# xp3i4/linear

Measured on AMD Instinct MI355X. Metric: reads/sec (whole node) + HBM GB/s on seed lookup, 10 kb reads vs GRCh38, higher is better.
Workload: dtype u64

## Files before the change

### linear_amd/csrc/lnr_api.hip

```cpp
#include <cstring>
#include <rocprim/device/device_radix_sort.hpp>
#include "lnr_kernels.hip"
#include "lnr_gap_args.h"
#include "../../include/linear_amd.h"

#include <algorithm>
#include <dlfcn.h>
#include <chrono>
#include <cstdio>
#include <cstdlib>
#include <atomic>
#include <condition_variable>
#include <deque>
#include <memory>
#include <mutex>
#include <string>
#include <thread>
#include <vector>

using namespace lnr;

#include "lnr_host_util.h"
#include "lnr_ctx.h"
#include "lnr_index.h"
// ... 176 lines not shown
        case LNR_ERR_NO_DEVICE: return "no usable HIP device (this library has no CPU path)";
        case LNR_ERR_HIP: return "HIP runtime error";
        case LNR_ERR_NOMEM: return "out of memory";
        case LNR_ERR_NO_INDEX: return "index not built";
        case LNR_ERR_LIMIT: return "input exceeds a format limit";
        case LNR_ERR_UNSUPPORTED: return "option not supported by this build";
        case LNR_ERR_INTERNAL: return "internal capacity overflow";
    }
    return "unknown status";
}
const char *lnr_last_error(const lnr_ctx *ctx) { return ctx ? const_cast<lnr_ctx *>(ctx)->err.show() : "null context"; }

lnr_status lnr_create(const lnr_opts *opts, lnr_ctx **out) {
    if (!out) return LNR_ERR_ARG;
    *out = nullptr;
    lnr_opts o;
    if (opts) o = *opts; else lnr_opts_default(&o);
    if ((o.index_type != 1 && o.index_type != 2) || o.feature_type != 2 || (o.preset != 1 && o.preset != 2) || o.dup > 1) return LNR_ERR_UNSUPPORTED;
    int ndev = 0;
    if (hipGetDeviceCount(&ndev) != hipSuccess || ndev <= 0) { (void)hipGetLastError(); return LNR_ERR_NO_DEVICE; }
    int dev = o.device;
    if (dev < 0) { if (hipGetDevice(&dev) != hipSuccess) return LNR_ERR_NO_DEVICE; }
    if (dev >= ndev) return LNR_ERR_ARG;
    int prev_dev = -1;
    (void)hipGetDevice(&prev_dev);
    if (hipSetDevice(dev) != hipSuccess) return LNR_ERR_NO_DEVICE;
    struct Restore { int d; ~Restore() { if (d >= 0) (void)hipSetDevice(d); } } restore_{prev_dev == dev ? -1 : prev_dev};
    lnr_ctx *ctx = new (std::nothrow) lnr_ctx();
    if (!ctx) return LNR_ERR_NOMEM;
    ctx->opts = o;
    ctx->device = dev;
    ctx->tun = tuning_from_env(dev);
    ctx->lane1_nomem_test = ctx->tun.lane1_nomem;
    ctx->lane[0] = lane_create(ctx, 0);
    bool ok = ctx->lane[0] && ctx->s_copy.create() && ctx->s_down.create() && ctx->ev_down.create() == hipSuccess && ctx->ev_done.create() == hipSuccess;
    if (!ok) { (void)hipGetLastError(); lnr_destroy(ctx); return LNR_ERR_HIP; }
    *out = ctx;
    return LNR_OK;
}

void lnr_destroy(lnr_ctx *ctx) {
    if (!ctx) return;
    (void)hipSetDevice(ctx->device);
    { std::lock_guard<std::mutex> g(ctx->mu); ctx->quit = true; }
    ctx->cv.notify_all();
    for (auto &L : ctx->lane) if (L && L->th.joinable()) L->th.join();
    ctx->s_copy.sync(); ctx->s_down.sync();
    delete ctx;
}

lnr_status lnr_filter_batch_dev(lnr_ctx *ctx, const uint8_t *d_reads, const uint64_t *d_off, uint32_t n, lnr_cords_dev *out) {
    if (!ctx || !d_off || (n && !d_reads)) return LNR_ERR_ARG;
    DevGuard dg_(ctx->device);
    if (in_flight(ctx)) { ctx->err = "batches submitted with lnr_filter_submit are still in flight"; return LNR_ERR_ARG; }
    return lane0_result(ctx, filter_dev(ctx->lane[0].get(), d_reads, d_off, n, out));
}
lnr_status lnr_last_gaps(lnr_ctx *ctx, lnr_gaps *out) {
    if (!ctx || !out) return LNR_ERR_ARG;
    DevGuard dg_(ctx->device);
    if (!ctx->tickets.empty()) { ctx->err = "lnr_last_gaps: batches are in flight (a worker is writing the per-read arrays)"; return LNR_ERR_ARG; }
    Lane *L = ctx->lane[0].get();
    u32 n = L->last_n;
    out->n_reads = n; out->n_gaps = 0; out->gap_off = nullptr; out->gaps = nullptr;
    ctx->h_gap_off.assign((size_t)n + 1, 0);
    ctx->h_gap_pairs.clear();
    if (n && L->last_gaps_off.size() == n) {
// ... 193 lines not shown
```

### linear_amd/csrc/lnr_ctx.h

```cpp
#pragma once
#include "lnr_handover.h"

struct lnr_ctx;

namespace {

struct Index {
    bool has_index = false;
    lnr_index_info info{};
    std::vector<u64> seq_len, seq_off, f2_off;
    u32 nbins = 0;
    DevBuf g, dir, hs, f2, d_seq_off, d_f2_off, d_seq_len;
    DevBuf bm, bl, ov;
    DevBuf hx_nkeys, hx_nvals; u32 hx_nnodes = 0; u64 hx_empty_dir = 0;
};

struct Tuning {
    size_t job_lds_bytes = 6 * 1024;
    u32 heavy_lds_kb = 48;
    u32 mid_cap = 6144, mid_lds_kb = 24;
    u32 heavy_cap = 0xffffffffu;
    u32 heavy_cap_r1 = 7000, mid_cap_r1 = 3000;
    u32 stop_after = 0;
    u32 mid_waves = 0;
    bool mid_cap_env = false;
    int seed_bm = -1;
    u32 prep_threads = 256;
    u32 prep_grid = 4096;
    u32 bulk_delay_ticks = 10000;
    u32 cap_shrink = 1;
    u32 seed_lds_pad = 0;
    u32 gap_arena2_mb = 64;
    u32 gap_teams = 96, ncu = 0;
    u32 gap_heavy_w = 60000;
    u64 gap_work_cap = 3000000;
    u32 nlanes = 2;
    int lane1_prio = 1;
    bool lane1_nomem = false;
    bool handover_gate = true;
    u64 gaps_spec = 0;
};

Tuning tuning_from_env(int device) {
    Tuning t;
    if (const char *e = getenv("LNR_LANES")) { long v = atol(e); if (v == 1 || v == 2) t.nlanes = (u32)v; }
    if (const char *e = getenv("LNR_LANE1_NOMEM")) t.lane1_nomem = atoi(e) != 0;
    if (const char *e = getenv("LNR_HANDOVER_GATE")) t.handover_gate = atoi(e) != 0;
    if (const char *e = getenv("LNR_GAPS_SPEC")) { long long v = atoll(e); if (v >= 1) t.gaps_spec = (u64)v; }
    if (const char *e = getenv("LNR_LANE1_PRIO")) { long v = atol(e); if (v >= -1 && v <= 1) t.lane1_prio = (int)v; }
    if (const char *e = getenv("LNR_CAP_SHRINK")) { long v = atol(e); if (v >= 1 && v <= 4096) t.cap_shrink = (u32)v; }
    if (const char *e = getenv("LNR_GAP_TEAMS")) { long v = atol(e); if (v >= 1 && v <= 4096) t.gap_teams = (u32)v; }
// ... 125 lines not shown
```

### linear_amd/csrc/lnr_hd.h

```cpp
#pragma once
#include <stdint.h>
#include <limits.h>
#include "ref_sort.h"

namespace lnr {

typedef uint64_t u64;
typedef int64_t i64;
typedef uint32_t u32;
typedef int32_t i32;
typedef uint16_t u16;
typedef uint8_t u8;

struct UP { u64 first, second; };

#if defined(__HIP_DEVICE_COMPILE__)
#define LNR_GLOBAL __attribute__((address_space(1)))
#define LNR_LDS __attribute__((address_space(3)))
#else
#define LNR_GLOBAL
#define LNR_LDS
#endif
template <class T> LNR_HD inline LNR_GLOBAL T *as_global(T *p) { return (LNR_GLOBAL T *)p; }
template <class T> LNR_HD inline LNR_LDS T *as_lds(T *p) { return (LNR_LDS T *)p; }

static const u64 ANCHOR_ZERO = 1ULL << 20;
static const u64 F_END = 1ULL << 60, F_STRAND = 1ULL << 61, F_RECD = 1ULL << 62, F_MAIN = 1ULL << 63;
static const u64 VALUE_MASK_DSTR = ((1ULL << 60) - 1) | F_STRAND;
static const u64 MAX_CORD_ID = (1ULL << 10) - 1, MAX_CORD_X = (1ULL << 30) - 1;

LNR_HD inline u64 cord_x(u64 v) { return (v >> 20) & ((1ULL << 30) - 1); }
LNR_HD inline u64 cord_y(u64 v) { return v & 0xfffffULL; }
LNR_HD inline u64 cord_strand(u64 v) { return (v >> 61) & 1ULL; }
LNR_HD inline u64 cord_id(u64 v) { return (v >> 50) & 1023ULL; }
LNR_HD inline u64 cord_x40(u64 v) { return (v >> 20) & 0xffffffffffULL; }
LNR_HD inline u64 mk_cord(u64 idx, u64 y, u64 s) { return (idx << 20) + y + (s << 61); }
// ... 13 lines not shown
}
LNR_HD inline UP forward_y(UP se, u64 L) {
    UP r;
    if (cord_strand(se.first)) { r.first = L - cord_y(se.second) - 1; r.second = L - cord_y(se.first) - 1; }
    else { r.first = cord_y(se.first); r.second = cord_y(se.second); }
    return r;
}

LNR_HD inline bool lnr_is_leader() {
#if defined(__HIP_DEVICE_COMPILE__)
    return (threadIdx.x & 63) == 0;
#else
    return true;
#endif
}
LNR_HD inline void lnr_wave_sync() {
#if defined(__HIP_DEVICE_COMPILE__)
    __builtin_amdgcn_fence(__ATOMIC_RELEASE, "workgroup");
    __builtin_amdgcn_wave_barrier();
    __builtin_amdgcn_fence(__ATOMIC_ACQUIRE, "workgroup");
#endif
}
LNR_HD inline u32 lnr_uni32(u32 v) {
#if defined(__HIP_DEVICE_COMPILE__)
    return (u32)__builtin_amdgcn_readfirstlane((int)v);
#else
    return v;
#endif
}
LNR_HD inline u64 lnr_uni64(u64 v) { return ((u64)lnr_uni32((u32)(v >> 32)) << 32) | (u64)lnr_uni32((u32)v); }
template <class T, class P = T *>
struct Vec {
    P p; u32 n, cap; int *ovf;
    LNR_HD void init(P p_, u32 cap_, int *ovf_) { p = p_; n = 0; cap = cap_; ovf = ovf_; }
    LNR_HD void push(const T &v) { if (n < cap) p[n++] = v; else *ovf = 1; }
    LNR_HD void push_u(const T &v) {
        if (n < cap) { if (lnr_is_leader()) p[n] = v; n++; }
        else if (lnr_is_leader()) *ovf = 1;
    }
    LNR_HD T &operator[](u32 i) { return p[i]; }
    LNR_HD T &back() { return p[n - 1]; }
};
struct Arena {
    char *base; u64 off, cap; int ovf; Arena *next;
    LNR_HD void init(void *b, u64 c) { base = (char *)b; off = 0; cap = c; ovf = 0; next = nullptr; }
    template <class T> LNR_HD T *get(u64 n) {
        u64 bytes = (n * sizeof(T) + 15) & ~15ULL;
        Arena *a = this;
        while (a->off + bytes > a->cap) {
            if (!a->next) { a->ovf = 1; ovf = 1; return (T *)base; }
            a = a->next;
        }
        T *r = (T *)(a->base + a->off);
        a->off += bytes;
        return r;
    }
};
struct Arena1 {
    char *base; u64 off, cap; int ovf;
    LNR_HD void init(void *b, u64 c) { base = (char *)b; off = 0; cap = c; ovf = 0; }
    template <class T> LNR_HD T *get(u64 n) {
        u64 bytes = (n * sizeof(T) + 15) & ~15ULL;
        if (off + bytes > cap) { ovf = 1; return (T *)base; }
        T *r = (T *)(base + off);
        off += bytes;
        return r;
    }
};
LNR_HD inline u64 job_scratch_bytes(u64 cap) { return (cap + 2) * 160 + 1024; }
LNR_HD inline u64 tail_scratch_bytes(u64 cap) { return cap * 240 + 8192; }

LNR_HD inline int lnr_popc64(u64 v) {
#if defined(__HIP_DEVICE_COMPILE__)
    return __popcll(v);
#else
    return __builtin_popcountll(v);
#endif
}
struct PackedSeq {
    const u64 *pk; const u32 *nm; u64 L;
    LNR_HD u8 operator[](u64 i) const {
        u64 j = i < L ? i : L;
        u32 n = nm[j >> 5]; u64 w = pk[j >> 5];
        u32 v = (u32)(w >> (2 * (j & 31))) & 3;
        return (u8)(((n >> (j & 31)) & 1) ? 4 : v);
    }
    LNR_HD int sum20(u64 p) const {
        u64 w = p >> 5; u32 sh = (u32)(p & 31);
// ... 873 lines not shown
#else
template <class FV, class CV>
LNR_HD inline bool extend_window(FV f1, FV f2, CV &cords, u64 &tail, u64 cordy_str, u64 cordy_end) {
    u32 p_str = cords.n - 1;
    u64 nc;
    while ((nc = previous_window(f1, f2, tail)) && cord_y(nc) >= cordy_str) {
        if (cords.n >= cords.cap) { *cords.ovf = 1; return false; }
        cords.push(nc); tail = nc;
    }
    u32 p_end = cords.n;
    if (p_end - p_str > 1) {
        for (u32 k = p_str; k < (p_str + p_end) / 2; k++) rs_swap(cords[k], cords[cords.n - k + p_str - 1]);
        tail = cords[cords.n - 1];
    }
    while ((nc = next_window(f1, f2, tail)) && cord_y(nc) + 96 < cordy_end) {
        if (cords.n >= cords.cap) { *cords.ovf = 1; return false; }
        cords.push(nc); tail = nc;
    }
    return true;
}
#endif
template <class FP, class OP> struct GenomeFeatT { FP base; OP off; u32 nseq; };
typedef GenomeFeatT<const F96 *, const u64 *> GenomeFeat;
typedef GenomeFeatT<LNR_GLOBAL const F96 *, LNR_GLOBAL const u64 *> GGenomeFeat;
template <class FP, class OP>
LNR_HD inline FeatViewT<FP> f2_view(GenomeFeatT<FP, OP> g, u64 id) {
    FeatViewT<FP> v;
    if (id >= g.nseq) { v.p = g.base; v.n = 0; return v; }
    v.p = g.base + g.off[id]; v.n = (u32)(g.off[id + 1] - g.off[id]);
    return v;
}
template <class FV, class GF>
LNR_HD inline void filter_hits_flags(const u64 *hits, u32 nhits, const FV f1[2], GF g, i32 *keep, u32 first, u32 step) {
    for (u32 it = 1 + first; it < nhits; it += step) {
        u32 dist = wdist_checked(f1[cord_strand(hits[it])], f2_view(g, cord_id(hits[it])), cord_y(hits[it]) >> 4, cord_x(hits[it]) >> 4);
        keep[it] = dist < 50 ? 1 : 0;
    }
}
LNR_HD inline u32 filter_hits_apply(u64 *hits, u32 nhits, const i32 *keep) {
    u32 mv = 0;
    for (u32 it = 1; it < nhits; it++) {
        if (keep[it]) hits[it - mv] = hits[it];
        else mv++;
        if (is_end(hits[it])) hits[it - mv] |= F_END;
    }
    return nhits - mv;
}
template <class FV, class GF, class CV>
LNR_HD inline void path_dst_2(const u64 *hits, u32 nhits, const FV f1_[2], GF g, CV &cords_, u64 read_str, u64 read_end, u64 L) {
    i64 hitBegin = 1, hitEnd = (i64)nhits;
    if (hitBegin >= hitEnd - 1) return;
    CV cords = cords_;
    struct NBack { CV &dst; CV &src; LNR_HD ~NBack() { dst.n = src.n; } } nback_{cords_, cords};
    FV f1[2] = {f1_[0], f1_[1]};
    cords.p = (decltype(cords.p))lnr_uni64((u64)cords.p); cords.n = lnr_uni32(cords.n); cords.cap = lnr_uni32(cords.cap); cords.ovf = (int *)lnr_uni64((u64)cords.ovf);
    for (int k = 0; k < 2; k++) { f1[k].p = (decltype(f1[k].p))lnr_uni64((u64)f1[k].p); f1[k].n = lnr_uni32(f1[k].n); }
    g.base = (decltype(g.base))lnr_uni64((u64)g.base); g.off = (decltype(g.off))lnr_uni64((u64)g.off); g.nseq = lnr_uni32(g.nseq);
    read_str = lnr_uni64(read_str); read_end = lnr_uni64(read_end); L = lnr_uni64(L);
    hitEnd = (i64)lnr_uni32(nhits);
    u64 tail;
    if (cords.n == 0) { cords.push_u(F_END); tail = F_END; }
    else tail = lnr_uni64(cords.p[cords.n - 1]);
    u64 ready_str, ready_end, cordy_str = 0, cordy_end = 0;
    bool f_sp_l, f_sp_r = false, f_block_end = false, f_append;
    i64 itt_next = hitBegin + 1, itt_first = hitBegin;
#if defined(LNR_PROF) && defined(__HIP_DEVICE_COMPILE__)
    unsigned long long pdc_[12] = {0, 0, 0, 0, 0, 0, 0, 0, 0, 0, 0, 0}, pdt_ = clock64();
    struct PdPrint { unsigned long long *c; u32 nh; __device__ ~PdPrint() { if ((blockIdx.x % 9973) == 777 && (threadIdx.x & 63) == 0)
        printf("[pd2] block %u: hits %u, visited %llu, extensions %llu, backward frontiers %llu (cords %llu, reversals %llu), forward frontiers %llu (cords %llu); cycles: hit walk %llu, backward %llu, reversal %llu, forward %llu\n",
               blockIdx.x, nh, c[10], c[0], c[1], c[3], c[5], c[2], c[4], c[9], c[6], c[7], c[8]); } } pdp_{pdc_, nhits};
#endif
#if defined(__HIP_DEVICE_COMPILE__)
    const u32 ln_ = threadIdx.x & 63;
    const u64 hreg0 = ln_ < nhits ? hits[ln_] : 0, hreg1 = ln_ + 64 < nhits ? hits[ln_ + 64] : 0;
    auto HIT = [&](i64 i) -> u64 {
        if (i < 128) {
            const u64 r = i < 64 ? hreg0 : hreg1;
            const int l_ = (int)(i & 63);
            return ((u64)(u32)__builtin_amdgcn_readlane((int)(u32)(r >> 32), l_) << 32) | (u64)(u32)__builtin_amdgcn_readlane((int)(u32)r, l_);
        }
        return lnr_uni64(hits[i]);
    };
#else
    auto HIT = [&](i64 i) -> u64 { return hits[i]; };
#endif
    u64 view_id = ~0ULL; FV view_f2; view_f2.p = g.base; view_f2.n = 0;
    for (i64 itt = hitBegin; itt < hitEnd; itt = itt_next++) {
        const u64 hi = HIT(itt), hpv = HIT(itt - 1);
        bool first_i = is_end(hpv);
// ... 2 lines not shown
        i64 da_l = first_i ? 0 : labs64((i64)(cord_x(hi) - cord_x(hpv) - cord_y(hi) + cord_y(hpv)));
        f_sp_l = (da_l > 80) || cord_strand(hi ^ hpv);
        while (1) {
            if (itt_next >= hitEnd) { f_block_end = true; itt_first = itt_next; break; }
            const u64 hn = HIT(itt_next), hp = HIT(itt_next - 1);
            if (is_end(hp)) { f_block_end = true; itt_first = itt_next; break; }
            i64 da_r = labs64((i64)(cord_x(hn) - cord_x(hp) - cord_y(hn) + cord_y(hp)));
            f_sp_r = (da_r > 80) || cord_strand(hn ^ hp);
            if ((cord_y(hi) + 96 < cord_y(hn) && cord_x(hi) + 96 < cord_x(hn)) || f_sp_r) break;
            itt_next++;
        }
        f_append = false;
        if (!f_sp_r && !f_block_end) {
            cordy_str = f_sp_l ? hi : (first_i ? ready_str : cord_y(tail));
            cordy_end = cord_y(HIT(itt_next));
            if (cords.n >= cords.cap) { if (lnr_is_leader()) *cords.ovf = 1; return; }
            cords.push_u(hi & ~F_END); tail = hi & ~F_END;
            f_append = true;
        } else {
            const u64 hl = HIT(itt_next - 1);
            if (!f_sp_l && cord_y(hl) >= 96 && cord_x(hl) >= 96) {
                u64 nc = shift_cord(hl, -96, -96);
                cordy_str = first_i ? read_str : cord_y(nc);
                cordy_end = cord_y(hl);
                if (cords.n >= cords.cap) { if (lnr_is_leader()) *cords.ovf = 1; return; }
                cords.push_u(nc & ~F_END); tail = nc & ~F_END;
                f_append = true;
            }
        }
        if (is_end(hi) || f_block_end) { f_block_end = true; cordy_end = ready_end; }
        if (f_append && cord_id(hi) != view_id) { view_id = cord_id(hi); view_f2 = f2_view(g, view_id); }
#if defined(LNR_PROF) && defined(__HIP_DEVICE_COMPILE__)
        { unsigned long long t_ = clock64(); pdc_[9] += t_ - pdt_; pdt_ = t_; pdc_[0] += f_append ? 1 : 0; pdc_[10]++; }
        if (f_append && !extend_window(f1[cord_strand(hi)], view_f2, cords, tail, cordy_str, cordy_end, pdc_)) return;
        pdt_ = clock64();
        if (0)
#endif
        if (f_append && !extend_window(f1[cord_strand(hi)], view_f2, cords, tail, cordy_str, cordy_end)) return;
        if (f_block_end) { tail |= F_END; if (lnr_is_leader()) cords.p[cords.n - 1] = tail; }
        itt_next = f_block_end ? itt_first : itt_next;
        f_sp_r = false; f_block_end = false;
    }
}

LNR_HD inline u32 clean_blocks(u64 *cords, u32 n, u64 drop_len) {
    if (n == 0) return 0;
    u64 ptr = 1, len = 0;
    for (u32 i = 1; i < n; i++) {
        len++;
        if (!is_end(cords[i - 1])) {
            i64 dx = (i64)(cord_x(cords[i]) - cord_x(cords[ptr - 1]));
            i64 dy = (i64)(cord_y(cords[i]) - cord_y(cords[ptr - 1]));
            if ((dx < 0 || dy < 0) && labs64(dx) < 50 && labs64(dy) < 50) { --len; --ptr; }
            else cords[ptr] = cords[i];
        } else cords[ptr] = cords[i];
        if (is_end(cords[i])) {
            ptr = len < drop_len ? ptr - len : ptr;
            len = 0;
            cords[ptr] |= F_END;
        }
        ptr++;
    }
    return (u32)ptr;
}
LNR_HD inline int gather_gaps_y(UP *str_ends, u32 ns, Vec<UP> &gaps, u64 L, u64 gap_size, LeaderScratch &ls) {
    u64 cord_frt = 0, cord_end = L - 1;
    int sum = 0;
    UP u;
    if (ns == 0) { u.first = cord_frt; u.second = cord_end; gaps.push(u); sum += (int)(cord_y(cord_end) - cord_y(cord_frt)); return sum; }
    ref_sort(str_ends, (long)ns, [L](const UP &i, const UP &j) {
        u64 y1 = cord_strand(i.first) ? L - cord_y(i.second) - 1 : cord_y(i.first);
// ... 88 lines not shown
        for (i32 j = ch.off[c]; j < ch.off[c + 1]; j++) len_current += ch.el[j].second - ch.el[j].first;
        if ((float)len_current > bound) {
            ++major_n;
            for (i32 j = ch.off[c]; j < ch.off[c + 1]; j++)
                for (u64 k = ch.el[j].first; k < ch.el[j].second; k++) out[n++] = hits[k] & ~F_END;
            out[n - 1] |= F_END;
        }
    }
    return n;
}

struct JobCtx {
    u64 L, read_str, read_end;
    int mode;
    GFeatView f1[2];
    GGenomeFeat g;
    u16 *bins; u32 nbins;
    u64 *pair_evals;
    unsigned long long *prof;
    int traceback_done;
};
struct JobScratch {
    Vec<u64> hits; Vec<i32> hscore; Vec<UP> sep, tmp;
    Rec rec;
    i32 *chain, *chain_sc, *cnt, *sep_score;
    u32 *xs, *ys;
    u64 *cuts, *xy_strs, *alt;
};
LNR_HD inline bool job_carve(Arena &ar, u32 cap, JobScratch &S, int *ovf) {
    u32 c2 = cap + 2;
    S.xs = ar.get<u32>(c2); S.ys = ar.get<u32>(c2);
    S.rec.score = ar.get<i32>(c2); S.rec.score2 = ar.get<i32>(c2); S.rec.len = ar.get<i32>(c2);
    S.rec.p2 = ar.get<i32>(c2); S.rec.root = ar.get<i32>(c2); S.rec.leaf = ar.get<i32>(c2);
    Arena &far_ = ar.next ? *ar.next : ar;
    S.hits.init(far_.get<u64>(c2), c2, ovf);
    S.hscore.init(far_.get<i32>(c2), c2, ovf);
    if (far_.ovf) ar.ovf = 1;
    S.cnt = ar.get<i32>(c2); S.chain = ar.get<i32>(c2); S.chain_sc = ar.get<i32>(c2);
    S.sep.init(ar.get<UP>(c2), c2, ovf);
    S.sep_score = ar.get<i32>(c2);
    S.tmp.init(ar.get<UP>(c2), c2, ovf);
    S.cuts = ar.get<u64>(2 * (u64)c2); S.xy_strs = ar.get<u64>(c2);
    return !ar.ovf;
}
struct JobDebug { u64 *filt; u32 *nfilt; u64 *xsort; u32 *nxsort; u64 *hits_chain; u32 *nhits_chain; u64 *hits_blocks; u32 *nhits_blocks; };

LNR_HD inline u32 job_phase1(u64 *a, u32 n_sorted, JobDebug *dbg, LeaderScratch &ls) {
    u32 m = n_sorted > 1 ? filter_anchor_list(a, n_sorted) : n_sorted;
    if (dbg && dbg->filt) { for (u32 i = 0; i < m; i++) dbg->filt[i] = a[i]; *dbg->nfilt = m; }
    ref_sort(a, (long)m, [](const u64 &p, const u64 &q) { return anchor_x(p) > anchor_x(q); }, ls.st);
    if (dbg && dbg->xsort) { for (u32 i = 0; i < m; i++) dbg->xsort[i] = a[i]; *dbg->nxsort = m; }
    return m;
}
LNR_HD inline void job_fill_xy(const u64 *a, u32 m, JobScratch &S, u32 first, u32 step) {
    for (u32 i = first; i < m; i += step) { S.xs[i] = (u32)anchor_x(a[i]); S.ys[i] = (u32)cord_y(a[i]); }
}

LNR_HD inline void job_blocks_gather(JobScratch &S, const JobCtx &c) {
    S.sep.n = 0; S.tmp.n = 0;
    gather_blocks(S.hits.p, S.hits.n, nullptr, S.sep, 1, S.hits.n, c.L, 600, 0, 0);
}
LNR_HD inline BlockScratch job_block_scratch(JobScratch &S, LeaderScratch &ls) {
    BlockScratch s; s.ptr = S.xs; s.sep_tmp = (UP *)S.cuts; s.score_tmp = (i32 *)S.ys; s.rec = S.rec; s.chain = S.chain_sc; s.chain_sc = (i32 *)S.xy_strs; s.cnt = S.cnt; s.ls = &ls;
    return s;
}
LNR_HD inline void job_blocks_scores(JobScratch &S, u32 first, u32 step) {
    for (u32 i = first; i < S.sep.n; i += step) S.sep_score[i] = S.hscore[(u32)S.sep[i].first] - S.hscore[(u32)S.sep[i].second - 1];
}
LNR_HD inline int job_blocks_finish(u64 *a, JobScratch &S, BlockSink &bs, JobDebug *dbg, u64 *&H, u32 &nH) {
    Vec<u64> &hits = S.hits;
// ... 104 lines not shown
```

### linear_amd/csrc/lnr_kernels.hip

```cpp
#pragma once
#include <hip/hip_runtime.h>
#include "lnr_hd.h"

namespace lnr {

}
#include "lnr_wave.h"
namespace lnr {

#define COPY_SEGS 8
struct CopySeg { const u32 *src; u32 *dst; u64 words; };
struct CopySegs { CopySeg s[COPY_SEGS]; u32 wg_end[COPY_SEGS]; u32 n; };
__global__ void __launch_bounds__(64) k_words_out(CopySegs S) {
    u32 b = blockIdx.x, k = 0;
    while (k + 1 < S.n && b >= S.wg_end[k]) k++;
    u32 w0 = k ? S.wg_end[k - 1] : 0, nwg = S.wg_end[k] - w0;
    const u32 *src = S.s[k].src; u32 *dst = S.s[k].dst; u64 n = S.s[k].words;
    for (u64 i = (u64)(b - w0) * 64 + threadIdx.x; i < n; i += (u64)nwg * 64) dst[i] = src[i];
}

#if defined(K_JOB_WAVES) && K_JOB_WAVES > 4
#define JOB_INLINE __forceinline__
#else
#define JOB_INLINE
#endif
#define SCAN_TPB 256
#define SCAN_IPT 16
#define SCAN_BLK (SCAN_TPB * SCAN_IPT)

__global__ void __launch_bounds__(SCAN_TPB) k_scan_blk(const i32 *in, i32 *out, u64 n, i32 *blk_sums) {
    __shared__ i32 sh[SCAN_TPB];
    u64 base = (u64)blockIdx.x * SCAN_BLK + (u64)threadIdx.x * SCAN_IPT;
    i32 v[SCAN_IPT];
    i32 sum = 0;
#pragma unroll
    for (int k = 0; k < SCAN_IPT; k++) { u64 idx = base + k; v[k] = idx < n ? in[idx] : 0; sum += v[k]; }
    sh[threadIdx.x] = sum;
    __syncthreads();
    for (int off = 1; off < SCAN_TPB; off <<= 1) {
        i32 t = threadIdx.x >= (unsigned)off ? sh[threadIdx.x - off] : 0;
        __syncthreads();
        sh[threadIdx.x] += t;
        __syncthreads();
    }
    i32 run = sh[threadIdx.x] - sum;
    if (threadIdx.x == SCAN_TPB - 1) blk_sums[blockIdx.x] = sh[SCAN_TPB - 1];
#pragma unroll
    for (int k = 0; k < SCAN_IPT; k++) { u64 idx = base + k; if (idx < n) out[idx] = run; run += v[k]; }
}
__global__ void __launch_bounds__(1024) k_scan_top(i32 *blk, u32 nblk) {
    __shared__ i32 sh[1024];
    __shared__ i32 carry;
    if (threadIdx.x == 0) carry = 0;
    __syncthreads();
// ... 2114 lines not shown
        if (lane < tn) { xi = xs[t0 + lane]; yi = ys[t0 + lane]; jl = jlo[t0 + lane]; }
        int lo = __builtin_amdgcn_readfirstlane(jl);
        T.wnear[wave][lane] = dp_before_tile<ST>(xs, ys, r.score, (int)t0, lo, xi, yi, jl, wave, NW);
        __syncthreads();
        if (wave == 0) {
            i64 best = -1;
#pragma unroll
            for (int w = 0; w < NW; w++) { i64 v = T.wnear[w][lane]; best = v > best ? v : best; }
            dp_in_tile_finish<ST>(T.tleaf, (int)t0, tn, xi, yi, jl, best, r);
        }
        __syncthreads();
    }
}
template <int NW>
__device__ void best_chains_block(const u32 *xs, const u32 *ys, u32 m, Rec r, int score_type, i32 *jlo, DpTile<NW> &T) {
    if (NW >= 8) {
        if (score_type) best_chains_block_t<NW, 1>(xs, ys, m, r, jlo, T);
        else best_chains_block_t<NW, 0>(xs, ys, m, r, jlo, T);
    } else {
        if (score_type) best_chains_block_flat<NW, 1>(xs, ys, m, r, jlo, T);
        else best_chains_block_flat<NW, 0>(xs, ys, m, r, jlo, T);
    }
}

struct DpShare { const u32 *xs, *ys; Rec rec; i32 *jlo; u32 m; int score_type; int abort; };
struct RadixShare { LNR_GLOBAL u64 *a, *alt; u32 n; };
#ifndef RADIX_BLOCK_MIN
#define RADIX_BLOCK_MIN 2048
#endif
struct SortShare { u64 *a; u32 *L, *R; u64 *tasks, *stg; u32 stg_cap, n; };
#ifndef SORT_BLOCK_MIN
#define SORT_BLOCK_MIN 2048
#endif
template <int NW>
__device__ __forceinline__ void job_group_run(const JobArgs &A, u32 grp, LNR_LDS u32 *dyn_lds) {
    __shared__ u32 s_m;
    __shared__ int s_ovf, s_flag[4];
    __shared__ u64 *s_H;
    __shared__ u32 s_nH, s_nhits;
    __shared__ LeaderScratch s_ls;
    static_assert(sizeof(s_ls.l_root) + sizeof(s_ls.l_score) + sizeof(s_ls.l_len) + sizeof(s_ls.l_leaf) == 256 * sizeof(u32), "tree tables = 256 words");
    LNR_LDS u32 *hist = as_lds((u32 *)s_ls.l_root);
    __shared__ DpTile<NW> s_tile;
    __shared__ DpShare s_dp;
    __shared__ RadixShare s_rs;
    __shared__ u32 s_rhist[NW > 1 ? NW : 1][256];
    __shared__ u32 s_rtot[NW > 1 ? 256 : 1], s_rflag;
    __shared__ SortShare s_so;
    __shared__ SortStack s_sstk[NW > 1 ? NW : 1];
    __shared__ SortDeferQ s_sq;
    int lane = lane_id();
    int wave = (int)(threadIdx.x >> 6);
    const bool lead = NW == 1 || wave == 0;
    u32 jb = A.grp_beg[grp], je = A.grp_beg[grp + 1];
    if (jb >= je) return;
    u32 r = A.J.read[jb];
    u64 L = A.read_len[r];
    if (threadIdx.x == 0) s_ovf = 0;
    if (NW == 1) WSYNC(); else __syncthreads();
    Vec<u64, LNR_GLOBAL u64 *> cords;
    cords.init(as_global(A.cords) + A.cords_off[r], A.cords_cap[r], &s_ovf);
    cords.n = A.ncords[r];
    unsigned long long tk_ = 0;
#ifdef LNR_PROF
    unsigned long long lnr_job_ph[16];
    for (int q = 0; q < 16; q++) lnr_job_ph[q] = 0;
    tk_ = clock64();
    unsigned long long *tl = (lead && lane == 0 && A.tl) ? A.tl + 4 * (size_t)(A.grp_lo + blockIdx.x) : nullptr;
    if (tl) { tl[0] = wall_clock64(); tl[2] = ((unsigned long long)__builtin_amdgcn_s_getreg(63508) << 32) | (unsigned)__builtin_amdgcn_s_getreg(63492); tl[3] = 0; }
#endif
    (void)tk_;
    unsigned long long *prof = (lead && lane == 0 && A.prof) ? A.prof + 32 * ((NW > 1 ? 2 : 0) + (A.J.mode[jb] ? 1 : 0)) : nullptr;
    (void)prof;
    for (u32 j = jb; j < je; j++) {
        u64 *a = nullptr;
        u32 m = 0;
        JobScratch S;
        int mode = (int)A.J.mode[j];
        Arena slow, ar;
        bool ok = true;
#ifdef LNR_PROF
        for (int q = 0; q < 16; q++) lnr_job_ph[q] = 0;
#endif
        LNR_GLOBAL u64 *ag = nullptr, *s_alt = nullptr;
        u32 n = 0, cap = 0;
        u32 *so_L = nullptr, *so_R = nullptr; u64 *so_tasks = nullptr, *so_stg = nullptr; u32 so_stg_cap = 0;
        if (lead) {
            ag = as_global(A.anchors) + A.anc_off[j];
            n = A.n_anchors[j];
            cap = n + 2;
            LNR_TICK(prof, 0, tk_);
            slow.init(A.scratch + A.scr_off[j], job_scratch_bytes(cap));
            LNR_GLOBAL u64 *alt = as_global(slow.get<u64>(cap));
            if (NW == 1 && A.stop_after == 1) break;
            n = binning_wave(ag, n, alt, dyn_lds, A.lds_bytes, A.nbins);
            LNR_TICK(prof, 1, tk_);
            if (NW == 1 && A.stop_after == 2) break;
            ar.init((void *)(u32 *)dyn_lds, A.arena_lds); ar.next = &slow;
            a = ag;
            if (n > 1) {
                s_alt = alt;
                a = ar.get<u64>((u64)n + 2);
                if (lane == 0) ag[0] = 0;
                WSYNC();
                if (NW == 1) radix_sort_wave(ag, alt, n, hist);
            }
        }
        if (NW > 1) {
            if (threadIdx.x == 0) { s_rs.a = ag; s_rs.alt = s_alt; s_rs.n = (n > 1 && n >= RADIX_BLOCK_MIN) ? n : 0; }
            __syncthreads();
            RadixShare rs = s_rs;
            if (rs.n) {
                if (NW >= 4) { [[clang::noinline]] radix_sort_block<NW>(rs.a, rs.alt, rs.n, as_lds(s_rhist), as_lds(s_rtot), as_lds(&s_rflag)); }
                else radix_sort_block<NW>(rs.a, rs.alt, rs.n, as_lds(s_rhist), as_lds(s_rtot), as_lds(&s_rflag));
            }
            else if (lead && n > 1) radix_sort_wave(ag, s_alt, n, hist);
        }
        if (lead) {
            if (n > 1) {
                for (u32 i = lane; i < n; i += 64) a[i] = ag[i];
                WSYNC();
            }
            LNR_TICK(prof, 2, tk_);
            if (NW == 1 && A.stop_after == 3) break;
            m = n > 1 ? filter_anchor_list_wave(a, n) : n;
            WSYNC();
            LNR_TICK(prof, 14, tk_);
            if (NW == 1 && A.stop_after == 13) break;
            if (m > 1) {
                so_L = (u32 *)(u64 *)s_alt; so_R = so_L + (m + 2);
                so_tasks = slow.get<u64>((u64)m + 2);
                {
                    bool a_in_lds = (char *)a >= (char *)(u32 *)dyn_lds && (char *)a < (char *)(u32 *)dyn_lds + A.arena_lds;
                    u64 used = (ar.off + 15) & ~15ULL;
                    if (!a_in_lds && A.arena_lds > used + 4096) { so_stg = (u64 *)((char *)(u32 *)dyn_lds + used); so_stg_cap = (u32)((A.arena_lds - used) / 8); }
                }
                if (NW == 1) introsort_xdesc_wave(a, m, so_L, so_R, so_tasks, &s_ls, so_stg, so_stg_cap);
            }
        }
        if (NW > 1) {
            if (threadIdx.x == 0) { s_so.a = a; s_so.L = so_L; s_so.R = so_R; s_so.tasks = so_tasks; s_so.stg = so_stg; s_so.stg_cap = so_stg_cap; s_so.n = (m > 1 && m >= SORT_BLOCK_MIN) ? m : 0; }
            __syncthreads();
            SortShare so = s_so;
            if (so.n) introsort_xdesc_block<NW>(so.a, so.n, so.L, so.R, so.tasks, s_sstk, &s_sq, so.stg, so.stg_cap);
            else if (lead && m > 1) introsort_xdesc_wave(a, m, so_L, so_R, so_tasks, &s_ls, so_stg, so_stg_cap);
        }
        if (lead) {
            LNR_TICK(prof, 15, tk_);
            if (NW == 1 && A.stop_after == 4) break;
            ok = job_carve(ar, m, S, &s_ovf) && !slow.ovf;
            if (ok) {
                job_fill_xy(a, m, S, (u32)lane, 64);
                WSYNC();
            } else if (lane == 0) s_ovf = 1;
            LNR_TICK(prof, 3, tk_);
        }
#ifdef LNR_PROF
        if (prof) {
            unsigned long long pairs = 0;
            if (ok && m >= 2) { u32 p300 = 0; for (u32 i = 0; i < m; i++) { while (p300 < i && S.xs[p300] - S.xs[i] >= 300) p300++; u32 js = i > 20 ? i - 20 : 0; pairs += i - (p300 < js ? p300 : js); } }
            if (tl) tl[3] += ((unsigned long long)m << 32) | (pairs > 0xffffffffULL ? 0xffffffffULL : pairs);
            lnr_job_ph[10] = m; lnr_job_ph[11] = pairs; lnr_job_ph[12] = A.n_anchors[j];
            atomicAdd(&prof[10], 1ULL); atomicAdd(&prof[11], (unsigned long long)m); atomicAdd(&prof[12], pairs); atomicAdd(&prof[13], (unsigned long long)A.n_anchors[j]);
            tk_ = clock64();
        }
#endif
        if (NW == 1) {
            if (!ok) break;
            if (m >= 2) {
                best_chains_wave(S.xs, S.ys, m, S.rec, job_parm(mode).score_type, S.cnt, s_tile.tleaf);
            }
        } else {
            if (threadIdx.x == 0) {
                s_dp.xs = S.xs; s_dp.ys = S.ys; s_dp.rec = S.rec; s_dp.jlo = S.cnt; s_dp.m = ok ? m : 0;
                s_dp.score_type = job_parm(mode).score_type; s_dp.abort = ok ? 0 : 1;
            }
            __syncthreads();
            DpShare d = s_dp;
            if (d.abort) break;
            if (d.m >= 2) best_chains_block<NW>(d.xs, d.ys, d.m, d.rec, d.score_type, d.jlo, s_tile);
        }
        LNR_TICK(prof, 4, tk_);
        if (NW == 1 && A.stop_after == 5) break;
        if (lead) {
            AnchorSink sink; sink.anchors = a; sink.hits = &S.hits; sink.hscore = &S.hscore; sink.first_len = 0; sink.nchains = 0;
            S.hits.n = 0; S.hscore.n = 0; S.hits.push_u(F_END); S.hscore.push_u(0);
            WSYNC();
            if (m >= 2) traceback_anchor_wave(S.rec, m, sink, S.chain, S.chain_sc, S.cnt, s_flag, &s_ls);
            LNR_TICK(prof, 5, tk_);
            if (NW == 1 && A.stop_after == 6) break;
            JobCtx c;
            c.traceback_done = 1;
            c.L = L; c.read_str = A.J.str[j]; c.read_end = A.J.end[j]; c.mode = mode;
            u32 nf = A.nf[r];
            c.f1[0].p = as_global(A.f1) + A.f1_off[r]; c.f1[0].n = nf;
            c.f1[1].p = as_global(A.f1) + A.f1_off[r] + nf; c.f1[1].n = nf;
            c.g.base = as_global(A.g.base); c.g.off = as_global(A.g.off); c.g.nseq = A.g.nseq; c.bins = nullptr; c.nbins = 0; c.pair_evals = nullptr; c.prof = prof;
            if (lane == 0) s_nhits = S.hits.n;
            WSYNC();
            S.hits.n = s_nhits;
            u64 *hits2 = a;
            const JobScratch S0 = S;
            u32 nb = 0;
            bool in_lds = false;
            if (A.arena_lds) {
                Arena pl; pl.init((void *)(u32 *)dyn_lds, A.arena_lds);
                const u32 nh = S.hits.n;
                u64 *lh = pl.get<u64>((u64)nh + 2), *lH = pl.get<u64>((u64)nh + 2);
                i32 *lcnt = pl.get<i32>((u64)nh + 2);
                u64 rest = pl.ovf ? 0 : A.arena_lds - pl.off;
                u32 C = rest > 14 * 16 + 2 * 100 ? (u32)((rest - 14 * 16) / 100) - 2 : 0;
                if (C >= 16) {
                    if (C > nh) C = nh;
                    if (lane == 0) s_flag[1] = 0;
                    for (u32 i = lane; i < nh; i += 64) lh[i] = S.hits.p[i];
                    S.hits.p = lh;
                    S.sep.init(pl.get<UP>((u64)C + 2), C, &s_flag[1]);
                    S.tmp.init(pl.get<UP>((u64)C + 2), C, &s_flag[1]);
                    S.cuts = pl.get<u64>(2 * (u64)C + 4); S.xy_strs = pl.get<u64>((u64)C + 2);
                    S.sep_score = pl.get<i32>((u64)C + 2);
                    S.xs = pl.get<u32>((u64)C + 2); S.ys = pl.get<u32>((u64)C + 2);
                    S.rec.score = pl.get<i32>((u64)C + 2); S.rec.score2 = pl.get<i32>((u64)C + 2); S.rec.len = pl.get<i32>((u64)C + 2);
                    S.rec.p2 = pl.get<i32>((u64)C + 2); S.rec.root = pl.get<i32>((u64)C + 2); S.rec.leaf = pl.get<i32>((u64)C + 2);
                    S.chain = pl.get<i32>((u64)C + 2); S.chain_sc = pl.get<i32>((u64)C + 2);
                    S.cnt = lcnt;
                    WSYNC();
                    if (!pl.ovf) {
                        nb = gather_blocks_wave(S.hits.p, nh, S.sep.p, S.sep.cap, S.sep.ovf);
                        bool fits = !s_flag[1];
                        if (fits) {
                            S.sep.n = nb;
                            nb = prefilter_chains2_wave(S.hits.p, nh, S.sep, nb, S.cuts, S.xy_strs, S.tmp, s_ls);
                            fits = !s_flag[1];
                        }
                        if (fits) { in_lds = true; hits2 = lH; }
                    }
                    if (!in_lds) { WSYNC(); S = S0; }
                }
            }
            if (!in_lds) {
                S.tmp.n = 0;
                nb = gather_blocks_wave(S.hits.p, S.hits.n, S.sep.p, S.sep.cap, S.sep.ovf);
                S.sep.n = nb;
                nb = prefilter_chains2_wave(S.hits.p, S.hits.n, S.sep, nb, S.cuts, S.xy_strs, S.tmp, s_ls);
            }
            S.sep.n = nb;
            LNR_TICK(prof, 6, tk_);
#ifdef LNR_PROF
            (void)in_lds;
            unsigned long long tsub_ = clock64();
#endif
            if (NW == 1 && A.stop_after == 7) break;
            job_blocks_scores(S, (u32)lane, 64);
            WSYNC();
            BlockScratch bsx = job_block_scratch(S, s_ls);
            if (nb >= 2) {
                chain_blocks_prepare_wave(S.hits.p, S.sep.p, S.sep_score, nb, bsx);
                if (NW == 1 && A.stop_after == 10) break;
#ifdef LNR_PROF
                unsigned long long tdp_ = clock64();
#endif
                best_chains2_wave(S.hits.p, bsx.sep_tmp, bsx.score_tmp, nb, bsx.rec, prof);
#ifdef LNR_PROF
                if (prof) atomicAdd(&prof[28], clock64() - tdp_);
#endif
                if (NW == 1 && A.stop_after == 11) break;
            }
#ifdef LNR_PROF
            tsub_ = clock64();
#endif
// ... 16 lines not shown
                    filter_hits_flags(H, nH, c.f1, c.g, S.cnt, (u32)lane, 64);
                    WSYNC();
                    if (lane == 0) s_nH = filter_hits_apply(H, nH, S.cnt);
                    WSYNC();
                    nH = s_nH;
                    LNR_TICK(prof, 8, tk_);
                    if (NW == 1 && A.stop_after == 9) break;
                    path_dst_2(H, nH, c.f1, c.g, cords, c.read_str, c.read_end, L);
                    LNR_TICK(prof, 9, tk_);
                }
            }
            WSYNC();
#ifdef LNR_PROF
            if (A.prof && lane == 0) {
                unsigned long long *mp = A.prof + 128 + 16 * ((NW > 1 ? 2 : 0) + (A.J.mode[jb] ? 1 : 0));
                unsigned long long old = atomicMax(&mp[10], lnr_job_ph[10]);
                if (lnr_job_ph[10] > old) { for (int q = 0; q < 10; q++) mp[q] = lnr_job_ph[q]; mp[11] = lnr_job_ph[11]; mp[12] = lnr_job_ph[12]; mp[14] = lnr_job_ph[14]; mp[15] = lnr_job_ph[15]; }
            }
            tk_ = clock64();
#endif
        }
        if (NW == 1) { if (s_ovf) break; }
        else {
            __syncthreads();
            if (s_ovf) break;
        }
    }
    if (lead && lane == 0) { A.ncords[r] = cords.n; if (s_ovf) A.read_err[r] = 1; }
#ifdef LNR_PROF
    if (tl) tl[1] = wall_clock64();
#endif
}

#ifndef K_JOB_WAVES
#define K_JOB_WAVES 4
#endif
__global__ void __attribute__((amdgpu_flat_work_group_size(64, 64), amdgpu_waves_per_eu(K_JOB_WAVES, K_JOB_WAVES))) k_job(JobArgs A) {
    extern __shared__ u32 dyn_lds[];
    if (A.grp_lo + blockIdx.x >= A.grp_hi) return;
    job_group_run<1>(A, A.grp_order[A.grp_lo + blockIdx.x], as_lds(dyn_lds));
}
__global__ void __launch_bounds__(1024) k_job_heavy(JobArgs A) {
    extern __shared__ u32 dyn_lds[];
    if (A.grp_lo + blockIdx.x >= A.grp_hi) return;
    job_group_run<16>(A, A.grp_order[A.grp_lo + blockIdx.x], as_lds(dyn_lds));
}
__global__ void __launch_bounds__(256, 4) k_job_mid(JobArgs A) {
    extern __shared__ u32 dyn_lds[];
    if (A.grp_lo + blockIdx.x >= A.grp_hi) return;
    job_group_run<4>(A, A.grp_order[A.grp_lo + blockIdx.x], as_lds(dyn_lds));
}
__global__ void __launch_bounds__(128, 4) k_job_mid2(JobArgs A) {
    extern __shared__ u32 dyn_lds[];
    if (A.grp_lo + blockIdx.x >= A.grp_hi) return;
    job_group_run<2>(A, A.grp_order[A.grp_lo + blockIdx.x], as_lds(dyn_lds));
}

__global__ void k_delay(unsigned ticks_100mhz) {
    unsigned long long t0 = wall_clock64();
    while (wall_clock64() - t0 < ticks_100mhz) __builtin_amdgcn_s_sleep(32);
}

struct TailArgs {
    const u32 *read_len; u32 n;
    const u32 *list;
    u64 *cords; const u64 *cords_off; const u32 *cords_cap; u32 *ncords; i32 *read_err;
    char *scratch; const u64 *scr_off; const u32 *scr_cap;
    UP *gaps; const u64 *gaps_off; const u32 *gaps_cap; u32 *ngaps; u32 *remap;
    UP *gdense; u32 *gcursor; u32 *gpos;
// ... 48 lines not shown
```

Baseline: 2.858 million.

## Raise k_job occupancy: five waves per EU, smaller LDS, leaner arena

The default k_job occupancy target goes from 4 to 5 waves per EU, which also turns on forced inlining. Default job LDS drops from 6 KB to 4 KB so more workgroups fit per CU. The linked-list Arena is replaced by a fast/far two-region arena, so the full JobScratch copy (S0) no longer needs saving and restoring in registers; on fallback the carve is redone from saved offsets. Shared-memory structs used only by multi-wave variants go into a struct that is empty for NW=1, and a debug occupancy print is added. The smaller LDS budget may push more work to global memory, and the tighter register limit may cause spills.

```diff
diff --git a/linear_amd/csrc/lnr_api.hip b/linear_amd/csrc/lnr_api.hip
--- a/linear_amd/csrc/lnr_api.hip
+++ b/linear_amd/csrc/lnr_api.hip
@@ -232,6 +232,12 @@
     ctx->device = dev;
     ctx->tun = tuning_from_env(dev);
     ctx->lane1_nomem_test = ctx->tun.lane1_nomem;
+    if (const char *e = getenv("LNR_DEBUG_OCC")) if (atoi(e)) {
+        size_t lds = (ctx->tun.job_lds_bytes + 15) & ~(size_t)15;
+        int nb = -1;
+        if (hipOccupancyMaxActiveBlocksPerMultiprocessor(&nb, lnr::k_job, 64, lds) != hipSuccess) { (void)hipGetLastError(); nb = -1; }
+        fprintf(stderr, "[lnr] k_job: %d workgroups per CU at %zu B of dynamic LDS\n", nb, lds);
+    }
     ctx->lane[0] = lane_create(ctx, 0);
     bool ok = ctx->lane[0] && ctx->s_copy.create() && ctx->s_down.create() && ctx->ev_down.create() == hipSuccess && ctx->ev_done.create() == hipSuccess;
     if (!ok) { (void)hipGetLastError(); lnr_destroy(ctx); return LNR_ERR_HIP; }
diff --git a/linear_amd/csrc/lnr_ctx.h b/linear_amd/csrc/lnr_ctx.h
--- a/linear_amd/csrc/lnr_ctx.h
+++ b/linear_amd/csrc/lnr_ctx.h
@@ -16,7 +16,7 @@
 };
 
 struct Tuning {
-    size_t job_lds_bytes = 6 * 1024;
+    size_t job_lds_bytes = 4 * 1024;
     u32 heavy_lds_kb = 48;
     u32 mid_cap = 6144, mid_lds_kb = 24;
     u32 heavy_cap = 0xffffffffu;
diff --git a/linear_amd/csrc/lnr_hd.h b/linear_amd/csrc/lnr_hd.h
--- a/linear_amd/csrc/lnr_hd.h
+++ b/linear_amd/csrc/lnr_hd.h
@@ -2,6 +2,12 @@
 #include <stdint.h>
 #include <limits.h>
 #include "ref_sort.h"
+
+#if defined(__HIPCC__)
+#define LNR_HD_FI __host__ __device__ __forceinline__
+#else
+#define LNR_HD_FI inline
+#endif
 
 namespace lnr {
 
@@ -81,9 +87,9 @@
 template <class T, class P = T *>
 struct Vec {
     P p; u32 n, cap; int *ovf;
-    LNR_HD void init(P p_, u32 cap_, int *ovf_) { p = p_; n = 0; cap = cap_; ovf = ovf_; }
+    LNR_HD_FI void init(P p_, u32 cap_, int *ovf_) { p = p_; n = 0; cap = cap_; ovf = ovf_; }
     LNR_HD void push(const T &v) { if (n < cap) p[n++] = v; else *ovf = 1; }
-    LNR_HD void push_u(const T &v) {
+    LNR_HD_FI void push_u(const T &v) {
         if (n < cap) { if (lnr_is_leader()) p[n] = v; n++; }
         else if (lnr_is_leader()) *ovf = 1;
     }
@@ -91,18 +97,25 @@
     LNR_HD T &back() { return p[n - 1]; }
 };
 struct Arena {
-    char *base; u64 off, cap; int ovf; Arena *next;
-    LNR_HD void init(void *b, u64 c) { base = (char *)b; off = 0; cap = c; ovf = 0; next = nullptr; }
-    template <class T> LNR_HD T *get(u64 n) {
-        u64 bytes = (n * sizeof(T) + 15) & ~15ULL;
-        Arena *a = this;
-        while (a->off + bytes > a->cap) {
-            if (!a->next) { a->ovf = 1; ovf = 1; return (T *)base; }
-            a = a->next;
-        }
-        T *r = (T *)(a->base + a->off);
-        a->off += bytes;
+    char *base; u64 off, cap; int ovf;
+    char *fbase; u64 foff, fcap;
+    LNR_HD_FI void init(void *b, u64 c) { base = (char *)b; off = 0; cap = c; ovf = 0; fbase = nullptr; foff = 0; fcap = 0; }
+    LNR_HD_FI void init_far(void *b, u64 c) { init(b, 0); fbase = (char *)b; fcap = c; }
+    LNR_HD_FI void set_fast(void *b, u64 c) { base = (char *)b; off = 0; cap = c; }
+    template <class T> LNR_HD_FI T *get_far(u64 n) {
+        u64 bytes = lnr_uni64((n * sizeof(T) + 15) & ~15ULL);
+        if (!fbase) return get<T>(n);
+        if (foff + bytes > fcap) { ovf = 1; return (T *)fbase; }
+        T *r = (T *)(fbase + foff);
+        foff += bytes;
         return r;
+    }
+    template <class T> LNR_HD_FI T *get(u64 n) {
+        u64 bytes = lnr_uni64((n * sizeof(T) + 15) & ~15ULL);
+        if (off + bytes <= cap) { T *r = (T *)(base + off); off += bytes; return r; }
+        if (fbase && foff + bytes <= fcap) { T *r = (T *)(fbase + foff); foff += bytes; return r; }
+        ovf = 1;
+        return (T *)base;
     }
 };
 struct Arena1 {
@@ -1042,8 +1055,9 @@
 }
 template <class FV, class GF>
 LNR_HD inline void filter_hits_flags(const u64 *hits, u32 nhits, const FV f1[2], GF g, i32 *keep, u32 first, u32 step) {
+    const FV f1a = f1[0], f1b = f1[1];
     for (u32 it = 1 + first; it < nhits; it += step) {
-        u32 dist = wdist_checked(f1[cord_strand(hits[it])], f2_view(g, cord_id(hits[it])), cord_y(hits[it]) >> 4, cord_x(hits[it]) >> 4);
+        u32 dist = wdist_checked(cord_strand(hits[it]) ? f1b : f1a, f2_view(g, cord_id(hits[it])), cord_y(hits[it]) >> 4, cord_x(hits[it]) >> 4);
         keep[it] = dist < 50 ? 1 : 0;
     }
 }
@@ -1062,9 +1076,10 @@
     if (hitBegin >= hitEnd - 1) return;
     CV cords = cords_;
     struct NBack { CV &dst; CV &src; LNR_HD ~NBack() { dst.n = src.n; } } nback_{cords_, cords};
-    FV f1[2] = {f1_[0], f1_[1]};
+    FV f1a = f1_[0], f1b = f1_[1];
     cords.p = (decltype(cords.p))lnr_uni64((u64)cords.p); cords.n = lnr_uni32(cords.n); cords.cap = lnr_uni32(cords.cap); cords.ovf = (int *)lnr_uni64((u64)cords.ovf);
-    for (int k = 0; k < 2; k++) { f1[k].p = (decltype(f1[k].p))lnr_uni64((u64)f1[k].p); f1[k].n = lnr_uni32(f1[k].n); }
+    f1a.p = (decltype(f1a.p))lnr_uni64((u64)f1a.p); f1a.n = lnr_uni32(f1a.n);
+    f1b.p = (decltype(f1b.p))lnr_uni64((u64)f1b.p); f1b.n = lnr_uni32(f1b.n);
     g.base = (decltype(g.base))lnr_uni64((u64)g.base); g.off = (decltype(g.off))lnr_uni64((u64)g.off); g.nseq = lnr_uni32(g.nseq);
     read_str = lnr_uni64(read_str); read_end = lnr_uni64(read_end); L = lnr_uni64(L);
     hitEnd = (i64)lnr_uni32(nhits);
@@ -1133,11 +1148,11 @@
         if (f_append && cord_id(hi) != view_id) { view_id = cord_id(hi); view_f2 = f2_view(g, view_id); }
 #if defined(LNR_PROF) && defined(__HIP_DEVICE_COMPILE__)
         { unsigned long long t_ = clock64(); pdc_[9] += t_ - pdt_; pdt_ = t_; pdc_[0] += f_append ? 1 : 0; pdc_[10]++; }
-        if (f_append && !extend_window(f1[cord_strand(hi)], view_f2, cords, tail, cordy_str, cordy_end, pdc_)) return;
+        if (f_append && !extend_window(cord_strand(hi) ? f1b : f1a, view_f2, cords, tail, cordy_str, cordy_end, pdc_)) return;
         pdt_ = clock64();
         if (0)
 #endif
-        if (f_append && !extend_window(f1[cord_strand(hi)], view_f2, cords, tail, cordy_str, cordy_end)) return;
+        if (f_append && !extend_window(cord_strand(hi) ? f1b : f1a, view_f2, cords, tail, cordy_str, cordy_end)) return;
         if (f_block_end) { tail |= F_END; if (lnr_is_leader()) cords.p[cords.n - 1] = tail; }
         itt_next = f_block_end ? itt_first : itt_next;
         f_sp_r = false; f_block_end = false;
@@ -1292,10 +1307,8 @@
     S.xs = ar.get<u32>(c2); S.ys = ar.get<u32>(c2);
     S.rec.score = ar.get<i32>(c2); S.rec.score2 = ar.get<i32>(c2); S.rec.len = ar.get<i32>(c2);
     S.rec.p2 = ar.get<i32>(c2); S.rec.root = ar.get<i32>(c2); S.rec.leaf = ar.get<i32>(c2);
-    Arena &far_ = ar.next ? *ar.next : ar;
-    S.hits.init(far_.get<u64>(c2), c2, ovf);
-    S.hscore.init(far_.get<i32>(c2), c2, ovf);
-    if (far_.ovf) ar.ovf = 1;
+    S.hits.init(ar.get_far<u64>(c2), c2, ovf);
+    S.hscore.init(ar.get_far<i32>(c2), c2, ovf);
     S.cnt = ar.get<i32>(c2); S.chain = ar.get<i32>(c2); S.chain_sc = ar.get<i32>(c2);
     S.sep.init(ar.get<UP>(c2), c2, ovf);
     S.sep_score = ar.get<i32>(c2);
diff --git a/linear_amd/csrc/lnr_kernels.hip b/linear_amd/csrc/lnr_kernels.hip
--- a/linear_amd/csrc/lnr_kernels.hip
+++ b/linear_amd/csrc/lnr_kernels.hip
@@ -19,7 +19,10 @@
     for (u64 i = (u64)(b - w0) * 64 + threadIdx.x; i < n; i += (u64)nwg * 64) dst[i] = src[i];
 }
 
-#if defined(K_JOB_WAVES) && K_JOB_WAVES > 4
+#ifndef K_JOB_WAVES
+#define K_JOB_WAVES 5
+#endif
+#if K_JOB_WAVES > 4
 #define JOB_INLINE __forceinline__
 #else
 #define JOB_INLINE
@@ -2200,6 +2203,16 @@
 #ifndef SORT_BLOCK_MIN
 #define SORT_BLOCK_MIN 2048
 #endif
+template <int NW> struct JobShare {
+    DpShare dp;
+    RadixShare rs;
+    u32 rhist[NW][256];
+    u32 rtot[256], rflag;
+    SortShare so;
+    SortStack sstk[NW];
+    SortDeferQ sq;
+};
+template <> struct JobShare<1> {};
 template <int NW>
 __device__ __forceinline__ void job_group_run(const JobArgs &A, u32 grp, LNR_LDS u32 *dyn_lds) {
     __shared__ u32 s_m;
@@ -2210,13 +2223,7 @@
     static_assert(sizeof(s_ls.l_root) + sizeof(s_ls.l_score) + sizeof(s_ls.l_len) + sizeof(s_ls.l_leaf) == 256 * sizeof(u32), "tree tables = 256 words");
     LNR_LDS u32 *hist = as_lds((u32 *)s_ls.l_root);
     __shared__ DpTile<NW> s_tile;
-    __shared__ DpShare s_dp;
-    __shared__ RadixShare s_rs;
-    __shared__ u32 s_rhist[NW > 1 ? NW : 1][256];
-    __shared__ u32 s_rtot[NW > 1 ? 256 : 1], s_rflag;
-    __shared__ SortShare s_so;
-    __shared__ SortStack s_sstk[NW > 1 ? NW : 1];
-    __shared__ SortDeferQ s_sq;
+    __shared__ JobShare<NW> s_sh;
     int lane = lane_id();
     int wave = (int)(threadIdx.x >> 6);
     const bool lead = NW == 1 || wave == 0;
@@ -2245,8 +2252,9 @@
         u32 m = 0;
         JobScratch S;
         int mode = (int)A.J.mode[j];
-        Arena slow, ar;
+        Arena ar;
         bool ok = true;
+        u64 carve_mark_off = 0, carve_mark_foff = 0;
 #ifdef LNR_PROF
         for (int q = 0; q < 16; q++) lnr_job_ph[q] = 0;
 #endif
@@ -2258,13 +2266,13 @@
             n = A.n_anchors[j];
             cap = n + 2;
             LNR_TICK(prof, 0, tk_);
-            slow.init(A.scratch + A.scr_off[j], job_scratch_bytes(cap));
-            LNR_GLOBAL u64 *alt = as_global(slow.get<u64>(cap));
+            ar.init_far(A.scratch + A.scr_off[j], job_scratch_bytes(cap));
+            LNR_GLOBAL u64 *alt = as_global(ar.get_far<u64>(cap));
             if (NW == 1 && A.stop_after == 1) break;
             n = binning_wave(ag, n, alt, dyn_lds, A.lds_bytes, A.nbins);
             LNR_TICK(prof, 1, tk_);
             if (NW == 1 && A.stop_after == 2) break;
-            ar.init((void *)(u32 *)dyn_lds, A.arena_lds); ar.next = &slow;
+            ar.set_fast((void *)(u32 *)dyn_lds, A.arena_lds);
             a = ag;
             if (n > 1) {
                 s_alt = alt;
@@ -2274,13 +2282,13 @@
                 if (NW == 1) radix_sort_wave(ag, alt, n, hist);
             }
         }
-        if (NW > 1) {
-            if (threadIdx.x == 0) { s_rs.a = ag; s_rs.alt = s_alt; s_rs.n = (n > 1 && n >= RADIX_BLOCK_MIN) ? n : 0; }
+        if constexpr (NW > 1) {
+            if (threadIdx.x == 0) { s_sh.rs.a = ag; s_sh.rs.alt = s_alt; s_sh.rs.n = (n > 1 && n >= RADIX_BLOCK_MIN) ? n : 0; }
             __syncthreads();
-            RadixShare rs = s_rs;
+            RadixShare rs = s_sh.rs;
             if (rs.n) {
-                if (NW >= 4) { [[clang::noinline]] radix_sort_block<NW>(rs.a, rs.alt, rs.n, as_lds(s_rhist), as_lds(s_rtot), as_lds(&s_rflag)); }
-                else radix_sort_block<NW>(rs.a, rs.alt, rs.n, as_lds(s_rhist), as_lds(s_rtot), as_lds(&s_rflag));
+                if (NW >= 4) { [[clang::noinline]] radix_sort_block<NW>(rs.a, rs.alt, rs.n, as_lds(s_sh.rhist), as_lds(s_sh.rtot), as_lds(&s_sh.rflag)); }
+                else radix_sort_block<NW>(rs.a, rs.alt, rs.n, as_lds(s_sh.rhist), as_lds(s_sh.rtot), as_lds(&s_sh.rflag));
             }
             else if (lead && n > 1) radix_sort_wave(ag, s_alt, n, hist);
         }
@@ -2297,7 +2305,7 @@
             if (NW == 1 && A.stop_after == 13) break;
             if (m > 1) {
                 so_L = (u32 *)(u64 *)s_alt; so_R = so_L + (m + 2);
-                so_tasks = slow.get<u64>((u64)m + 2);
+                so_tasks = ar.get_far<u64>((u64)m + 2);
                 {
                     bool a_in_lds = (char *)a >= (char *)(u32 *)dyn_lds && (char *)a < (char *)(u32 *)dyn_lds + A.arena_lds;
                     u64 used = (ar.off + 15) & ~15ULL;
@@ -2306,17 +2314,18 @@
                 if (NW == 1) introsort_xdesc_wave(a, m, so_L, so_R, so_tasks, &s_ls, so_stg, so_stg_cap);
             }
         }
-        if (NW > 1) {
-            if (threadIdx.x == 0) { s_so.a = a; s_so.L = so_L; s_so.R = so_R; s_so.tasks = so_tasks; s_so.stg = so_stg; s_so.stg_cap = so_stg_cap; s_so.n = (m > 1 && m >= SORT_BLOCK_MIN) ? m : 0; }
+        if constexpr (NW > 1) {
+            if (threadIdx.x == 0) { s_sh.so.a = a; s_sh.so.L = so_L; s_sh.so.R = so_R; s_sh.so.tasks = so_tasks; s_sh.so.stg = so_stg; s_sh.so.stg_cap = so_stg_cap; s_sh.so.n = (m > 1 && m >= SORT_BLOCK_MIN) ? m : 0; }
             __syncthreads();
-            SortShare so = s_so;
-            if (so.n) introsort_xdesc_block<NW>(so.a, so.n, so.L, so.R, so.tasks, s_sstk, &s_sq, so.stg, so.stg_cap);
+            SortShare so = s_sh.so;
+            if (so.n) introsort_xdesc_block<NW>(so.a, so.n, so.L, so.R, so.tasks, s_sh.sstk, &s_sh.sq, so.stg, so.stg_cap);
             else if (lead && m > 1) introsort_xdesc_wave(a, m, so_L, so_R, so_tasks, &s_ls, so_stg, so_stg_cap);
         }
         if (lead) {
             LNR_TICK(prof, 15, tk_);
             if (NW == 1 && A.stop_after == 4) break;
-            ok = job_carve(ar, m, S, &s_ovf) && !slow.ovf;
+            carve_mark_off = ar.off; carve_mark_foff = ar.foff;
+            ok = job_carve(ar, m, S, &s_ovf);
             if (ok) {
                 job_fill_xy(a, m, S, (u32)lane, 64);
                 WSYNC();
@@ -2333,18 +2342,18 @@
             tk_ = clock64();
         }
 #endif
-        if (NW == 1) {
+        if constexpr (NW == 1) {
             if (!ok) break;
             if (m >= 2) {
                 best_chains_wave(S.xs, S.ys, m, S.rec, job_parm(mode).score_type, S.cnt, s_tile.tleaf);
             }
         } else {
             if (threadIdx.x == 0) {
-                s_dp.xs = S.xs; s_dp.ys = S.ys; s_dp.rec = S.rec; s_dp.jlo = S.cnt; s_dp.m = ok ? m : 0;
-                s_dp.score_type = job_parm(mode).score_type; s_dp.abort = ok ? 0 : 1;
+                s_sh.dp.xs = S.xs; s_sh.dp.ys = S.ys; s_sh.dp.rec = S.rec; s_sh.dp.jlo = S.cnt; s_sh.dp.m = ok ? m : 0;
+                s_sh.dp.score_type = job_parm(mode).score_type; s_sh.dp.abort = ok ? 0 : 1;
             }
             __syncthreads();
-            DpShare d = s_dp;
+            DpShare d = s_sh.dp;
             if (d.abort) break;
             if (d.m >= 2) best_chains_block<NW>(d.xs, d.ys, d.m, d.rec, d.score_type, d.jlo, s_tile);
         }
@@ -2368,7 +2377,7 @@
             WSYNC();
             S.hits.n = s_nhits;
             u64 *hits2 = a;
-            const JobScratch S0 = S;
+            const u32 nhs0 = S.hscore.n;
             u32 nb = 0;
             bool in_lds = false;
             if (A.arena_lds) {
@@ -2403,7 +2412,12 @@
                         }
                         if (fits) { in_lds = true; hits2 = lH; }
                     }
-                    if (!in_lds) { WSYNC(); S = S0; }
+                    if (!in_lds) {
+                        WSYNC();
+                        ar.off = carve_mark_off; ar.foff = carve_mark_foff;
+                        job_carve(ar, m, S, &s_ovf);
+                        S.hits.n = nh; S.hscore.n = nhs0;
+                    }
                 }
             }
             if (!in_lds) {
@@ -2486,9 +2500,6 @@
 #endif
 }
 
-#ifndef K_JOB_WAVES
-#define K_JOB_WAVES 4
-#endif
 __global__ void __attribute__((amdgpu_flat_work_group_size(64, 64), amdgpu_waves_per_eu(K_JOB_WAVES, K_JOB_WAVES))) k_job(JobArgs A) {
     extern __shared__ u32 dyn_lds[];
     if (A.grp_lo + blockIdx.x >= A.grp_hi) return;
```

Result: faster. 2.951 million, median of 6 (+3.3%).
